# sonniki/image-captioning-with-external-knowledge

Hardware: AMD Instinct MI355X
Metric: decode_steps_per_sec (higher is better)
Workload: dtype f32 (3xbf16 split products, fp32 accumulate); 1 GPU; cfg2: geo variant, per-GPU batch 64 x 20 decode positions, 14x14x2048 features, K=20 knowledge rows, vocab 10000; global_batch=64, graph=True, collective_backend=none, split_allreduce=False, parallelism=dp1 (one flat-bucket all-reduce per step)

## Files before the change

### image-captioning-with-external-knowledge_amd/csrc/attention_mfma.hip

```cpp
#include <algorithm>

#include "attention_mfma.h"

#ifdef ICK_ATTN_STAMPS
__device__ unsigned long long ick_attn_stamps[4][16];
#define ICK_ASTAMP(kern, i)                                                                   \
    do {                                                                                      \
        if (threadIdx.x == 0 && blockIdx.x == 0 && blockIdx.y == 0) ick_attn_stamps[kern][i] = __builtin_readcyclecounter(); \
    } while (0)
extern "C" int ick_debug_read_attn_stamps(unsigned long long* out) {
    return (int)hipMemcpyFromSymbol(out, HIP_SYMBOL(ick_attn_stamps), sizeof(ick_attn_stamps));
}
#else
#define ICK_ASTAMP(kern, i)
#endif

namespace ick {
namespace {

constexpr int DHP = 32;
constexpr int QLD = DHP + 4;

__device__ __forceinline__ float4 mask_cols(float4 x, int c0, int dh) {
    x.x = c0 + 0 < dh ? x.x : 0.f; x.y = c0 + 1 < dh ? x.y : 0.f;
    x.z = c0 + 2 < dh ? x.z : 0.f; x.w = c0 + 3 < dh ? x.w : 0.f;
    return x;
}

__device__ __forceinline__ int wave_id_of(unsigned tid) { return __builtin_amdgcn_readfirstlane((int)(tid >> 6)); }

__device__ __forceinline__ f32x4 mfma4(const float4& a, const float4& b, f32x4 c) {
    c = __builtin_amdgcn_mfma_f32_16x16x4f32(a.x, b.x, c, 0, 0, 0);
    c = __builtin_amdgcn_mfma_f32_16x16x4f32(a.y, b.y, c, 0, 0, 0);
// ... 161 lines not shown
        }
        if (lq == 0) rsum[wave * NQ + 16 * qt + li] = sum[qt];
    }
    ICK_ASTAMP(SK, 6);
    __syncthreads();
    ICK_ASTAMP(SK, 7);
#pragma unroll
    for (int qt = 0; qt < NQT; ++qt)
#pragma unroll
        for (int jt = 0; jt < 2; ++jt)
            *reinterpret_cast<f32x4*>(Ored + ((wave * NQT + qt) * 2 + jt) * 256 + lane * 4) = oacc[qt][jt];
    if (tid < NQ) {
        const float s = (rsum[tid] + rsum[NQ + tid]) + (rsum[2 * NQ + tid] + rsum[3 * NQ + tid]);
        stat[NQ + tid] = s > 0.f ? 1.f / s : 0.f;
        if (p.lse && tid < T) p.lse[((int64_t)b * p.H + h) * T + tid] = stat[tid] + __logf(s);
    }
    __syncthreads();
    for (int tt = wave; tt < NQT * 2; tt += 4) {
        const int qt = tt >> 1, jt = tt & 1;
        f32x4 o = {0.f, 0.f, 0.f, 0.f};
#pragma unroll
        for (int w = 0; w < 4; ++w) o += *reinterpret_cast<const f32x4*>(Ored + ((w * NQT + qt) * 2 + jt) * 256 + lane * 4);
        const int query = 16 * qt + li;
        if (query < T) {
            const float inv = stat[NQ + query];
            float* orow = p.O + (int64_t)b * p.o_bs + (int64_t)query * p.o_ts + h * dh;
            const int j0 = 16 * jt + 4 * lq;
#pragma unroll
            for (int r = 0; r < 4; ++r)
                if (j0 + r < dh) orow[j0 + r] = o[r] * inv;
        }
    }
    ICK_ASTAMP(SK, 8);
}

template <int NQT, int MAXT>
__global__ __launch_bounds__(256) void attn_bwd_mfma_kernel(ick_attn_bwd_args p, int SP, bool st2) {
    chain_priority_bwd();
    [[maybe_unused]] constexpr int SK = MAXT > 1 ? 3 : 2;
    ICK_ASTAMP(SK, 0);
    constexpr int NQ = NQT * 16;
    constexpr int TLD = NQ + 4;
    extern __shared__ __attribute__((aligned(16))) float smem[];
    const int TR = (p.T + 3) & ~3;
    float* dSs = smem;
    float* Qs = dSs + TR * SP;
    float* Gs = Qs + NQ * QLD;
    float* Qt = Gs + NQ * QLD;
    float* Gt = Qt + DHP * TLD;
    float* Ls = Gt + DHP * TLD;
    float* Dl = Ls + NQ;
    float* Kw = Dl + NQ + (wave_id_of(threadIdx.x)) * (16 * QLD);
    float* dQp = Qs;

    const int b = blockIdx.x, h = blockIdx.y;
    const int tid = threadIdx.x, lane = tid & 63, wave = tid >> 6;
    const int li = lane & 15, lq = lane >> 4;
    const int T = p.T, S = p.S, dh = p.dh;
    const int nkt = (S + 15) >> 4;
    const Dropout drop = make_dropout(p.drop_p, epoch_seed(p.drop_seed, p.drop_epoch), p.drop_site);
    const float* qb = p.Q + (int64_t)b * p.q_bs + (int64_t)h * p.q_hs;
    const float* kb = p.K + (int64_t)b * p.k_bs + (int64_t)h * p.k_hs;
    const float* vb = p.V + (int64_t)b * p.v_bs + (int64_t)h * p.v_hs;
    const float* ob = p.O + (int64_t)b * p.o_bs + h * dh;
    const float* gb = p.dO + (int64_t)b * p.o_bs + h * dh;

    constexpr int QIT = (NQ * 8 + 255) / 256;
    float4 qx[QIT];
#pragma unroll
    for (int it = 0; it < QIT; ++it) {
        const int f = tid + 256 * it;
        const int t = f >> 3, c = f & 7;
        qx[it] = *reinterpret_cast<const float4*>(qb + (int64_t)(t < T ? t : 0) * DHP + 4 * c);
    }
    const float lse_v = p.lse[((int64_t)b * p.H + h) * T + (tid < T ? tid : 0)];
    float gv[NQT * 2], ov[NQT * 2];
#pragma unroll
    for (int it = 0; it < NQT * 2; ++it) {
        const int f = tid + 256 * it;
        const int t = f >> 5, j = f & 31;
        const bool ok = t < T && j < dh;
        const int64_t at = ok ? (int64_t)t * p.o_ts + j : 0;
        gv[it] = gb[at];
        ov[it] = ob[at];
    }
    float4 kf[MAXT][2], vf[MAXT][2];
#pragma unroll
    for (int i = 0; i < MAXT; ++i) {
        const int key = 16 * (wave + 4 * i) + li;
        const int64_t ro = (int64_t)(key < S ? key : 0) * DHP + 4 * lq;
#pragma unroll
        for (int t = 0; t < 2; ++t) {
            kf[i][t] = *reinterpret_cast<const float4*>(kb + ro + 16 * t);
            vf[i][t] = *reinterpret_cast<const float4*>(vb + ro + 16 * t);
        }
    }
    ICK_ASTAMP(SK, 1);
#pragma unroll
    for (int it = 0; it < QIT; ++it) {
        const int f = tid + 256 * it;
        const int t = f >> 3, c = f & 7;
        if (f < NQ * 8) {
            const float4 x = mask_cols(qx[it], 4 * c, t < T ? dh : 0);
            *reinterpret_cast<float4*>(Qs + t * QLD + 4 * c) = x;
            Qt[(4 * c + 0) * TLD + t] = x.x; Qt[(4 * c + 1) * TLD + t] = x.y;
            Qt[(4 * c + 2) * TLD + t] = x.z; Qt[(4 * c + 3) * TLD + t] = x.w;
        }
    }
#pragma unroll
    for (int it = 0; it < NQT * 2; ++it) {
        const int f = tid + 256 * it;
        const int t = f >> 5, j = f & 31;
        const bool ok = t < T && j < dh;
        const float g = ok ? gv[it] : 0.f, o = ok ? ov[it] : 0.f;
        Gs[t * QLD + j] = g;
        Gt[j * TLD + t] = g;
        float d = g * o;
        d += __shfl_xor(d, 1, 64); d += __shfl_xor(d, 2, 64); d += __shfl_xor(d, 4, 64);
        d += __shfl_xor(d, 8, 64); d += __shfl_xor(d, 16, 64);
        if (j == 0) Dl[t] = d;
    }
    if (tid < NQ) Ls[tid] = tid < T ? lse_v : 0.f;
    ICK_ASTAMP(SK, 2);
    __syncthreads();
    ICK_ASTAMP(SK, 3);

    f32x4 dq[NQT][2];
#pragma unroll
    for (int qt = 0; qt < NQT; ++qt)
#pragma unroll
        for (int jt = 0; jt < 2; ++jt) dq[qt][jt] = f32x4{0.f, 0.f, 0.f, 0.f};
#pragma unroll
    for (int i = 0; i < MAXT; ++i) {
        const int kt = wave + 4 * i;
        if (kt >= nkt) continue;
        const int key = 16 * kt + li;
        const bool kok = key < S;
#pragma unroll
        for (int t = 0; t < 2; ++t) {
            kf[i][t] = mask_cols(kf[i][t], 16 * t + 4 * lq, kok ? dh : 0);
            vf[i][t] = mask_cols(vf[i][t], 16 * t + 4 * lq, kok ? dh : 0);
        }
#pragma unroll
        for (int t = 0; t < 2; ++t) *reinterpret_cast<float4*>(Kw + li * QLD + 16 * t + 4 * lq) = kf[i][t];
        f32x4 dvt[2] = {{0.f, 0.f, 0.f, 0.f}, {0.f, 0.f, 0.f, 0.f}};
        f32x4 dkt[2] = {{0.f, 0.f, 0.f, 0.f}, {0.f, 0.f, 0.f, 0.f}};
#pragma unroll
        for (int qt = 0; qt < NQT; ++qt) {
            f32x4 s = {0.f, 0.f, 0.f, 0.f}, dp = {0.f, 0.f, 0.f, 0.f};
#pragma unroll
            for (int t = 0; t < 2; ++t) {
                const float4 qa = *reinterpret_cast<const float4*>(Qs + (16 * qt + li) * QLD + 16 * t + 4 * lq);
                const float4 ga = *reinterpret_cast<const float4*>(Gs + (16 * qt + li) * QLD + 16 * t + 4 * lq);
                s = mfma4(qa, kf[i][t], s);
                dp = mfma4(ga, vf[i][t], dp);
            }
            const float4 l4 = *reinterpret_cast<const float4*>(Ls + 16 * qt + 4 * lq);
            const float4 d4 = *reinterpret_cast<const float4*>(Dl + 16 * qt + 4 * lq);
            const float lr[4] = {l4.x, l4.y, l4.z, l4.w}, dr[4] = {d4.x, d4.y, d4.z, d4.w};
            float pd[4], ds[4];
#pragma unroll
            for (int r = 0; r < 4; ++r) {
                const int query = 16 * qt + 4 * lq + r;
                float pr = __expf(s[r] * p.scale - lr[r]);
                if (!kok || query >= T || (p.causal && key > p.q_pos0 + query)) pr = 0.f;
                float mk = 1.f;
                if (drop.on()) mk = drop.mask((uint32_t)((b * p.H + h) * T + query) * (uint32_t)S + (uint32_t)key);
                ds[r] = pr * (dp[r] * mk - dr[r]) * p.scale;
                pd[r] = pr * mk;
                if (query < T) dSs[query * SP + key] = ds[r];
            }
            const float4 pf = make_float4(pd[0], pd[1], pd[2], pd[3]);
            const float4 df = make_float4(ds[0], ds[1], ds[2], ds[3]);
#pragma unroll
            for (int jt = 0; jt < 2; ++jt) {
                const float4 gt = *reinterpret_cast<const float4*>(Gt + (16 * jt + li) * TLD + 16 * qt + 4 * lq);
                const float4 qt4 = *reinterpret_cast<const float4*>(Qt + (16 * jt + li) * TLD + 16 * qt + 4 * lq);
                dvt[jt] = mfma4(gt, pf, dvt[jt]);
                dkt[jt] = mfma4(qt4, df, dkt[jt]);
            }
        }
        __builtin_amdgcn_fence(__ATOMIC_RELEASE, "wavefront");
        __builtin_amdgcn_wave_barrier();
        {
            float4 kq[2];
#pragma unroll
            for (int jt = 0; jt < 2; ++jt) {
                const float* kc = Kw + (4 * lq) * QLD + 16 * jt + li;
                kq[jt] = make_float4(kc[0], kc[QLD], kc[2 * QLD], kc[3 * QLD]);
            }
#pragma unroll
            for (int qt = 0; qt < NQT; ++qt) {
                const float4 da = *reinterpret_cast<const float4*>(dSs + (16 * qt + li) * SP + 16 * kt + 4 * lq);
#pragma unroll
                for (int jt = 0; jt < 2; ++jt) dq[qt][jt] = mfma4(da, kq[jt], dq[qt][jt]);
            }
        }
        __builtin_amdgcn_wave_barrier();
        if (kok) {
            float* dvr = p.dV + (int64_t)b * p.dv_bs + (int64_t)key * p.dv_ss + h * dh;
            float* dkr = p.dK + (int64_t)b * p.dk_bs + (int64_t)key * p.dk_ss + h * dh;
#pragma unroll
            for (int jt = 0; jt < 2; ++jt) {
                const int j0 = 16 * jt + 4 * lq;
                if (st2) {
                    if (j0 + 1 < dh) {
                        *reinterpret_cast<float2*>(dvr + j0) = make_float2(dvt[jt][0], dvt[jt][1]);
                        *reinterpret_cast<float2*>(dkr + j0) = make_float2(dkt[jt][0], dkt[jt][1]);
                    }
                    if (j0 + 3 < dh) {
                        *reinterpret_cast<float2*>(dvr + j0 + 2) = make_float2(dvt[jt][2], dvt[jt][3]);
                        *reinterpret_cast<float2*>(dkr + j0 + 2) = make_float2(dkt[jt][2], dkt[jt][3]);
                    }
                } else {
#pragma unroll
                    for (int r = 0; r < 4; ++r)
                        if (j0 + r < dh) { dvr[j0 + r] = dvt[jt][r]; dkr[j0 + r] = dkt[jt][r]; }
                }
            }
        }
    }
    ICK_ASTAMP(SK, 4);
    __syncthreads();
    ICK_ASTAMP(SK, 5);
#pragma unroll
    for (int qt = 0; qt < NQT; ++qt)
#pragma unroll
        for (int jt = 0; jt < 2; ++jt)
            *reinterpret_cast<f32x4*>(dQp + ((wave * NQT + qt) * 2 + jt) * 256 + lane * 4) = dq[qt][jt];
    __syncthreads();
    for (int tt = wave; tt < NQT * 2; tt += 4) {
        const int qt = tt >> 1, jt = tt & 1;
        const int j = 16 * jt + li;
        f32x4 acc = {0.f, 0.f, 0.f, 0.f};
#pragma unroll
        for (int w = 0; w < 4; ++w) acc += *reinterpret_cast<const f32x4*>(dQp + ((w * NQT + qt) * 2 + jt) * 256 + lane * 4);
        if (j < dh) {
#pragma unroll
            for (int r = 0; r < 4; ++r) {
                const int query = 16 * qt + 4 * lq + r;
                if (query < T) p.dQ[(int64_t)b * p.dq_bs + (int64_t)query * p.dq_ts + h * dh + j] = acc[r];
            }
        }
    }
    ICK_ASTAMP(SK, 6);
}

template <int NQT, int MAXT>
int launch_fwd(const ick_attn_args& a, int SP, hipStream_t s) {
    const size_t fl = std::max<size_t>((size_t)DHP * SP, 4 * NQT * 2 * 256) + (size_t)NQT * 16 * QLD + 10 * NQT * 16;
    if (fl * sizeof(float) > 150 * 1024) return kAttnMfmaUnsupported;
    auto kern = attn_fwd_mfma_kernel<NQT, MAXT>;
    static LdsAttrOnce attr;
    if (int e = attr.ensure((const void*)kern, 160 * 1024)) return e;
    hipLaunchKernelGGL(kern, dim3(a.H, a.B), dim3(256), fl * sizeof(float), s, a, SP);
    ICK_LAUNCH_RET();
}

template <int NQT, int MAXT>
int launch_bwd(const ick_attn_bwd_args& a, int SP, hipStream_t s) {
    constexpr int NQ = NQT * 16;
    const size_t tr = (size_t)((a.T + 3) & ~3);
    const size_t fl = std::max(tr * SP + 2 * (size_t)NQ * QLD + 2 * (size_t)DHP * (NQ + 4) + 2 * NQ + 4 * 16 * QLD,
                               (size_t)NQ * SP + 64);
    if (fl * sizeof(float) > 150 * 1024) return kAttnMfmaUnsupported;
    auto kern = attn_bwd_mfma_kernel<NQT, MAXT>;
    static LdsAttrOnce attr;
    if (int e = attr.ensure((const void*)kern, 160 * 1024)) return e;
    const bool st2 = a.dh % 2 == 0 && a.dk_bs % 2 == 0 && a.dk_ss % 2 == 0 && a.dv_bs % 2 == 0 && a.dv_ss % 2 == 0 &&
// ... 49 lines not shown
```

### image-captioning-with-external-knowledge_amd/csrc/common.h

```cpp
#pragma once
#include <hip/hip_runtime.h>
#include <stdint.h>
#include <stdlib.h>

#include "ick_amd.h"

namespace ick {

using f32x4 = __attribute__((ext_vector_type(4))) float;

constexpr int kWave = 64;

inline int ceil_div(int64_t a, int64_t b) { return (int)((a + b - 1) / b); }

extern int g_deterministic;
inline bool deterministic() {
    if (g_deterministic < 0) {
        const char* e = getenv("ICK_DETERMINISTIC");
        g_deterministic = (e && e[0] && e[0] != '0') ? 1 : 0;
    }
    return g_deterministic == 1;
}

#define ICK_CHECK_ARG(cond)          \
// ... 94 lines not shown
    uint32_t thr, seed, site;
    float scale;
    __device__ __forceinline__ bool on() const { return thr != 0u; }
    __device__ __forceinline__ float mask(uint32_t idx) const { return drop_hash(seed, site, idx) >= thr ? scale : 0.f; }
};
__host__ __device__ __forceinline__ Dropout make_dropout(float p, uint32_t seed, uint32_t site) {
    Dropout d{0u, seed, site, 1.f};
    if (p > 0.f) {
        d.thr = (uint32_t)fminf(p * 4294967296.f, 4294967040.f);
        d.scale = 1.f / (1.f - p);
    }
    return d;
}
__device__ __forceinline__ uint32_t epoch_seed(uint32_t seed, const uint32_t* epoch) {
    if (epoch == nullptr) return seed;
#if defined(__HIP_DEVICE_COMPILE__)
    uint32_t v;
    asm volatile("s_load_dword %0, %1, 0x0\n\ts_waitcnt lgkmcnt(0)" : "=s"(v) : "s"(epoch) : "memory");
    return seed + v;
#else
    return seed + *epoch;
#endif
}
__device__ __forceinline__ int device_bound(int host, const int32_t* dev) {
    if (dev == nullptr) return host;
#if defined(__HIP_DEVICE_COMPILE__)
    int v;
    asm volatile("s_load_dword %0, %1, 0x0\n\ts_waitcnt lgkmcnt(0)" : "=s"(v) : "s"(dev) : "memory");
    return min(host, max(v, 0));
#else
    return host;
#endif
}
__device__ __forceinline__ int clamp_row(int64_t v, int n) {
    return (int)(v < 0 ? 0 : (v >= (int64_t)n ? (int64_t)n - 1 : v));
}
constexpr int kRuleHistMax = 128;
__device__ __forceinline__ uint4 rule_words(const int32_t* words) {
    if (words == nullptr) return make_uint4(0u, 0u, 0u, 0u);
#if defined(__HIP_DEVICE_COMPILE__)
    uint64_t w01;
    uint32_t w2;
    asm volatile("s_load_dwordx2 %0, %2, 0x0\n\ts_load_dword %1, %2, 0x8\n\ts_waitcnt lgkmcnt(0)"
                 : "=&s"(w01), "=&s"(w2) : "s"(words) : "memory");
    return make_uint4((uint32_t)w01, (uint32_t)(w01 >> 32), w2, 0u);
#else
    return make_uint4((uint32_t)words[0], (uint32_t)words[1], (uint32_t)words[2], (uint32_t)words[3]);
#endif
}

template <typename Tok>
__device__ __forceinline__ void mark_bans(const Tok* hist, int t, int n, int m, int end_token, uint32_t* bits, int c0,
                                          int nwords, int* hs) {
    const int tid = threadIdx.x, nt = blockDim.x;
    for (int w = tid; w < nwords; w += nt) bits[w] = 0u;
    if (n > 0)
        for (int p = tid; p < t; p += nt) hs[p] = (int)hist[p];
    __syncthreads();
    if (n > 0) {
        for (int p = n - 1 + tid; p < t; p += nt) {
            bool match = true;
            for (int j = 1; j < n; ++j) match = match && hs[p - j] == hs[t - j];
            const int c = hs[p] - c0;
            if (match && c >= 0 && c < 32 * nwords) atomicOr(&bits[c >> 5], 1u << (c & 31));
        }
    }
// ... 41 lines not shown
```

### image-captioning-with-external-knowledge_amd/lib.py

```python
import ctypes as C
import os

_PKG = os.path.dirname(os.path.abspath(__file__))
LIB_PATH = os.path.join(_PKG, "libick_amd.so")
if os.environ.get("ICK_LIB_PATH"):
    LIB_PATH = os.environ["ICK_LIB_PATH"]

ICK_GEO, ICK_KNOWLEDGE, ICK_NEWS = 0, 1, 2
VARIANT_ID = {"geo": ICK_GEO, "knowledge": ICK_KNOWLEDGE, "news": ICK_NEWS}
GEMM_RELU, GEMM_ACCUM, GEMM_ATOMIC, GEMM_COLSUM_ONLY = 1, 2, 4, 16

vp = C.c_void_p
i32 = C.c_int32
i64 = C.c_int64
f32 = C.c_float
u32 = C.c_uint32


class GemmArgs(C.Structure):
    _fields_ = [
        ("A", vp), ("B", vp), ("C", vp), ("bias", vp),
        ("M", i32), ("N", i32), ("K", i32),
        ("a_rs", i64), ("a_ks", i64), ("a_grp", i32), ("a_gs", i64), ("a_gmap", vp),
        ("b_rs", i64), ("b_ks", i64),
# ... 64 lines not shown

class AdamBlock(C.Structure):
    _fields_ = [("item", i32), ("tn", i32), ("tk", i32), ("cnt4", i32), ("off4", i64), ("copy", vp)]


class LrSchedule(C.Structure):
    _fields_ = [("kind", i32), ("warmup", i32), ("total", i32), ("min_ratio", f32)]


OPT_WORDS = 8
LR_KINDS = {"constant": 0, "inverse_sqrt": 1, "cosine": 2, "linear": 3}


class AttnArgs(C.Structure):
    _fields_ = [
        ("Q", vp), ("K", vp), ("V", vp), ("O", vp), ("lse", vp),
        ("B", i32), ("H", i32), ("T", i32), ("S", i32), ("dh", i32),
        ("q_bs", i64), ("q_hs", i64), ("q_ts", i64), ("k_bs", i64), ("k_hs", i64), ("k_ss", i64),
        ("v_bs", i64), ("v_hs", i64), ("v_ss", i64), ("o_bs", i64), ("o_ts", i64),
        ("scale", f32), ("causal", i32), ("q_pos0", i32), ("kv_len", vp),
        ("drop_p", f32), ("drop_seed", u32), ("drop_site", u32), ("drop_epoch", vp),
    ]


class AttnBwdArgs(C.Structure):
    _fields_ = [
        ("Q", vp), ("K", vp), ("V", vp), ("O", vp), ("dO", vp), ("lse", vp), ("dQ", vp), ("dK", vp), ("dV", vp),
        ("B", i32), ("H", i32), ("T", i32), ("S", i32), ("dh", i32),
        ("q_bs", i64), ("q_hs", i64), ("q_ts", i64), ("k_bs", i64), ("k_hs", i64), ("k_ss", i64),
        ("v_bs", i64), ("v_hs", i64), ("v_ss", i64), ("o_bs", i64), ("o_ts", i64),
        ("dq_bs", i64), ("dq_ts", i64), ("dk_bs", i64), ("dk_ss", i64), ("dv_bs", i64), ("dv_ss", i64),
        ("scale", f32), ("causal", i32), ("q_pos0", i32),
        ("drop_p", f32), ("drop_seed", u32), ("drop_site", u32), ("drop_epoch", vp),
    ]


class DecodeLayer(C.Structure):
    _fields_ = [(n, vp) for n in ("sa_in_w", "sa_in_b", "sa_out_wt", "sa_out_b", "n1_g", "n1_b",
                                  "ca_in_w", "ca_in_b", "ca_out_wt", "ca_out_b", "n2_g", "n2_b",
                                  "w1", "b1", "w2t", "b2", "n3_g", "n3_b", "self_k", "self_v", "cross_k", "cross_v")]


MAX_LAYERS = 8


class DecodeCtx(C.Structure):
    _fields_ = ([(n, i32) for n in ("R", "rows_per_sample", "d", "H", "FF", "layers", "S", "max_len", "V", "K", "F",
                                    "end_token", "pad_token")] +
                [("ln_eps", f32), ("emb_scale", f32), ("kv_bs", i64), ("scores_ld", i64),
                 ("layer", DecodeLayer * MAX_LAYERS)] +
                [(n, vp) for n in ("anc", "wv", "bv", "we", "be", "wf", "bf", "ee", "fe", "gate", "eib", "word_emb", "pe",
                                   "x0", "xa", "xb", "xc", "p1", "p2", "p3", "hfin", "hv", "ptr", "cand", "scores",
                                   "output", "hist", "finished", "n_done", "next_token", "next_mask", "cap_buf", "sel_state")])


class BeamState(C.Structure):
    _fields_ = [(n, vp) for n in ("cum", "fin", "seq_in", "seq_out", "anc_in", "anc_out", "cap_in", "cap_out", "rec")] + \
               [("start_token", i32)]


class SampleState(C.Structure):
    _fields_ = [(n, vp) for n in ("seed", "temp_top_p", "top_k", "log_prob")]


class DecodeRules(C.Structure):
    _fields_ = [(n, vp) for n in ("words", "lp", "len")]
# ... 136 lines not shown
```

### image-captioning-with-external-knowledge_amd/ops.py

```python
import contextlib
import ctypes as C
import gc
import math
import os

import torch

from . import lib as L


def _p(t):
    return None if t is None else t.data_ptr()


def _stream():
    return torch.cuda.current_stream().cuda_stream


def _f32c(t, name):
    if t.dtype != torch.float32 or not t.is_cuda:
        raise L.IckError("%s must be a float32 device tensor (got %s on %s)" % (name, t.dtype, t.device))
    return t


# ... 841 lines not shown
    N = rouge_l.shape[0] if rouge_l.dim() == 1 else -1
    if N < 1 or tuple(counts.shape) != (N, 10) or tuple(pointers.shape) != (N, 3):
        raise L.IckError("caption_metric_sums needs counts (N, 10), rouge_l (N,) and pointers (N, 3), N >= 1")
    dev = counts.device
    if out is None:
        out = (torch.empty(14, device=dev, dtype=torch.int64), torch.empty(1, device=dev, dtype=torch.float64))
    sums, rouge_sum = out
    assert sums.shape == (14,) and sums.dtype == torch.int64 and sums.is_contiguous()
    assert rouge_sum.shape == (1,) and rouge_sum.dtype == torch.float64
    L.check(L.load().ick_caption_metric_sums(_p(counts), _p(rouge_l), _p(pointers), N, _p(sums), _p(rouge_sum),
                                             _p(sums[13:14]), _stream()), "ick_caption_metric_sums")
    return sums, rouge_sum


def attention_bwd_buffer(shape, T, S, dh, device):
    if L.load().ick_attention_bwd_overwrites(T, S, dh):
        return torch.empty(shape, device=device, dtype=torch.float32)
    return torch.zeros(shape, device=device, dtype=torch.float32)


ATTN_PLAN_KEYS = ("mfma", "nqt", "maxt", "dhp", "tq", "chunks", "overwrites")


def attention_plan(direction, T, S, dh, head_major=True):
    out = (C.c_int32 * len(ATTN_PLAN_KEYS))()
    rc = L.load_raw().ick_attention_plan({"fwd": 0, "bwd": 1}[direction], T, S, dh, int(head_major), out)
    if rc == -1:
        return None
    L.check(rc, "ick_attention_plan")
    return dict(zip(ATTN_PLAN_KEYS, (int(v) for v in out)))


def attention_heads_bwd(q, kv, O, dO, lse, dQ, dK, dV, H, dh, T, S, q_seg=0, k_seg=0, v_seg=1, causal=False,
                        drop=None, q_pos0=0):
    B = q.shape[0]
    Tq, Sa = q.shape[3], kv.shape[3]
    hp = q.shape[4]
    assert kv.shape[4] == hp
    a = L.AttnBwdArgs()
    a.Q = q.data_ptr() + 4 * (q_seg * H * Tq * hp)
    a.K = kv.data_ptr() + 4 * (k_seg * H * Sa * hp)
    a.V = kv.data_ptr() + 4 * (v_seg * H * Sa * hp)
    a.O, a.dO, a.lse = _p(O), _p(dO), _p(lse)
    a.dQ, a.dK, a.dV = _p(dQ), _p(dK), _p(dV)
    a.B, a.H, a.T, a.S, a.dh = B, H, T, S, dh
    a.q_bs, a.q_hs, a.q_ts = q.stride(0), Tq * hp, hp
    a.k_bs, a.k_hs, a.k_ss = kv.stride(0), Sa * hp, hp
    a.v_bs, a.v_hs, a.v_ss = kv.stride(0), Sa * hp, hp
    a.o_bs, a.o_ts = O.stride(0), O.stride(1)
    a.dq_bs, a.dq_ts = dQ.stride(0), dQ.stride(1)
    a.dk_bs, a.dk_ss = dK.stride(0), dK.stride(1)
    a.dv_bs, a.dv_ss = dV.stride(0), dV.stride(1)
    a.scale = 1.0 / math.sqrt(dh)
    a.causal, a.q_pos0 = int(causal), q_pos0
    _drop(a, drop)
    L.check(L.load().ick_attention_bwd(C.byref(a), _stream()), "ick_attention_bwd")


def layernorm_bwd(dy, x, res, gamma, mean, rstd, dgamma, dbeta, drop=None):
    d = x.shape[-1]
    rows = x.numel() // d
    dz = torch.empty_like(x)
    dxd = torch.empty_like(x)
    rpb = L.load().ick_layernorm_bwd_rows_per_block()
    part = torch.empty((rows + rpb - 1) // rpb, 2 * d, device=x.device, dtype=torch.float32)
    L.check(L.load().ick_layernorm_bwd(_p(dy), _p(x), _p(res), _p(gamma), _p(mean), _p(rstd), _p(dz), None, None,
                                       rows, d, _p(dxd), *_dargs(drop), _p(part), _stream()), "ick_layernorm_bwd")

    if SIDE is not None:
        SIDE.flush()
    ln_partials_reduce(part, dgamma, dbeta)
    return dz, dxd


def ln_partials_reduce(part, dgamma, dbeta):
    d = part.shape[1] // 2
    adjacent = dbeta.data_ptr() == dgamma.data_ptr() + 4 * d
    if SIDE is not None:
        if adjacent:
            SIDE.add_problem(colsum_problem(part, dgamma), part)
        else:
            SIDE.add_problem(colsum_problem(part[:, :d], dgamma), part)
            SIDE.add_problem(colsum_problem(part[:, d:], dbeta), part)
    elif adjacent:
        colsum(part, dgamma, n_out=2 * d)
    else:
        colsum(part[:, :d], dgamma)
        colsum(part[:, d:], dbeta)
# ... 350 lines not shown
```

### image-captioning-with-external-knowledge_amd/training.py

```python
import functools
import math
import os
import weakref

import torch

from . import dp, ops
from .decoder import DropSites
from .lib import IckError
from .weights import DerivedWeights, first_stage, vocab_planes_wanted


class Tape:

    def __init__(self):
        self.enc_layers = {}
        self.dec_layers = []
        self.misc = {}


def _p(x):
    return x.detach()


# ... 219 lines not shown
                _lin_bwd(grads, dqkv.view(M, 3 * d), t["x"].view(M, d), layer.self_attn.in_proj_weight,
                         layer.self_attn.in_proj_bias, need_dx=False)
                dz, g0, w0p = dz_out, dqkv.view(M, 3 * d), pkb[(tag, li, "siT")]
            else:
                dx = _lin_bwd(grads, dqkv.view(M, 3 * d), t["x"].view(M, d), layer.self_attn.in_proj_weight,
                              layer.self_attn.in_proj_bias, dx=dz_out, acc=True).view(B, T, d)
                if ops.SIDE is not None:
                    ops.SIDE.flush_group_here()
        return dx
    for layer, t in zip(reversed(layers), reversed(tapes)):
        B, T, _ = t["x"].shape
        M = B * T
        dz, do2 = ops.layernorm_bwd(dx, t["o2"], t["x1"], _p(layer.norm2.weight), t["m2"], t["r2"],
                                    _g(grads, layer.norm2.weight), _g(grads, layer.norm2.bias), drop=t["d2"])
        dpre = _lin_bwd(grads, do2.view(M, d), t["f"].view(M, -1), layer.linear2.weight, layer.linear2.bias,
                        gate=t["f"].view(M, -1), gate_scale=_keep_scale(t["d_ff"]))
        dx1 = _lin_bwd(grads, dpre, t["x1"].view(M, d), layer.linear1.weight, layer.linear1.bias, dx=dz.view(M, d),
                       acc=True)
        dz, do1 = ops.layernorm_bwd(dx1.view(B, T, d), t["o1"], t["x"], _p(layer.norm1.weight), t["m1"], t["r1"],
                                    _g(grads, layer.norm1.weight), _g(grads, layer.norm1.bias), drop=t["d1"])
        dsa = _lin_bwd(grads, do1.view(M, d), t["sa"].view(M, d), layer.self_attn.out_proj.weight,
                       layer.self_attn.out_proj.bias)
        dqkv = ops.attention_bwd_buffer((B, T, 3 * d), T, T, d // H, dx.device)
        ops.attention_heads_bwd(t["qkv"], t["qkv"], t["sa"], dsa.view(B, T, d), t["lse"], dqkv[:, :, :d],
                                dqkv[:, :, d:2 * d], dqkv[:, :, 2 * d:], H, d // H, T, T, 0, 1, 2, drop=t["d_att"])
        dx = _lin_bwd(grads, dqkv.view(M, 3 * d), t["x"].view(M, d), layer.self_attn.in_proj_weight,
                      layer.self_attn.in_proj_bias, dx=dz.view(M, d), acc=True).view(B, T, d)
        if ops.SIDE is not None:
            ops.SIDE.flush_group()
    return dx


def _decoder_layer_bwd_chain(dec, li, layer, t, state, dkv_rows, kv, S, grads, pkb, mem2=None, mem_t_ps=None,
                             valid=None):
    H, d = dec.num_heads, dec.emb_dim
    dh = d // H
    B, T, _ = t["x"].shape
    M = B * T
    dev = t["x"].device
    dz, g0, w0p = state
    n3 = _norm_args(t, 3, t["x2"], layer.norm3, grads, M, d, dev)
    n2 = _norm_args(t, 2, t["x1"], layer.norm2, grads, M, d, dev)
    dpre = torch.empty(M, layer.linear1.out_features, device=dev, dtype=torch.float32)
    dca = torch.empty(M, d, device=dev, dtype=torch.float32)
    dz_a = torch.empty(M, d, device=dev, dtype=torch.float32)
    ops.rowchain_bwd(M, d, n3, pkb[("d", li, "coT")], dca, dz_a, g0=g0, w0p=w0p, dzin=dz,
                     ffn=dict(w1p=pkb[("d", li, "l2T")], w2p=pkb[("d", li, "l1T")], act=t["f"],
                              gate_scale=_keep_scale(t["d_ff"]), t_out=dpre), norm2=n2)
    if ops.SIDE is not None:
        ops.SIDE.flush()
    ops.ln_partials_reduce(n3["part"], _g(grads, layer.norm3.weight), _g(grads, layer.norm3.bias))
    ops.ln_partials_reduce(n2["part"], _g(grads, layer.norm2.weight), _g(grads, layer.norm2.bias))
    _lin_bwd(grads, n3["do"], t["f"].view(M, -1), layer.linear2.weight, layer.linear2.bias, need_dx=False,
             valid=valid)
    _lin_bwd(grads, dpre, t["x2"].view(M, d), layer.linear1.weight, layer.linear1.bias, need_dx=False, valid=valid)
    _lin_bwd(grads, n2["do"], t["ca"].view(M, d), layer.multihead_attn.out_proj.weight,
             layer.multihead_attn.out_proj.bias, need_dx=False, valid=valid)
    if ops.SIDE is not None:
        ops.SIDE.flush_group()
    dq = torch.empty(B, T, d, device=dev, dtype=torch.float32)
    c0 = 2 * li * d
    ops.attention_heads_bwd(t["qc"], kv, t["ca"], dca.view(B, T, d), t["lse_c"], dq, dkv_rows[:, :, c0:c0 + d],
                            dkv_rows[:, :, c0 + d:c0 + 2 * d], H, dh, T, S, 0, 2 * li, 2 * li + 1, drop=t["d_ca"])
    if ops.SIDE is not None:
        ops.SIDE.flush()
    if mem2 is not None:
        _kv_proj_param_grads(layer, li, dkv_rows, mem2, grads, d, mem_t_ps)
    n1 = _norm_args(t, 1, t["x"], layer.norm1, grads, M, d, dev)
    dsa = torch.empty(M, d, device=dev, dtype=torch.float32)
    dz_b = torch.empty(M, d, device=dev, dtype=torch.float32)
    ops.rowchain_bwd(M, d, n1, pkb[("d", li, "soT")], dsa, dz_b, g0=dq.view(M, d), w0p=pkb[("d", li, "cqT")], dzin=dz_a)
    if ops.SIDE is not None:
        ops.SIDE.flush()
    ops.ln_partials_reduce(n1["part"], _g(grads, layer.norm1.weight), _g(grads, layer.norm1.bias))
    _lin_bwd(grads, dq.view(M, d), t["x1"].view(M, d), layer.multihead_attn.in_proj_weight,
             layer.multihead_attn.in_proj_bias, w_rows=slice(0, d), need_dx=False, valid=valid)
    _lin_bwd(grads, n1["do"], t["sa"].view(M, d), layer.self_attn.out_proj.weight, layer.self_attn.out_proj.bias,
             need_dx=False, valid=valid)
    dqkv = ops.attention_bwd_buffer((B, T, 3 * d), T, T, dh, dev)
    ops.attention_heads_bwd(t["qkv"], t["qkv"], t["sa"], dsa.view(B, T, d), t["lse_s"], dqkv[:, :, :d],
                            dqkv[:, :, d:2 * d], dqkv[:, :, 2 * d:], H, dh, T, T, 0, 1, 2, causal=True,
                            drop=t["d_sa"])
    if li > 0:
        _lin_bwd(grads, dqkv.view(M, 3 * d), t["x"].view(M, d), layer.self_attn.in_proj_weight,
                 layer.self_attn.in_proj_bias, need_dx=False, valid=valid)
        out = (dz_b, dqkv.view(M, 3 * d), pkb[("d", li, "siT")])
    else:
        dx0 = _lin_bwd(grads, dqkv.view(M, 3 * d), t["x"].view(M, d), layer.self_attn.in_proj_weight,
                       layer.self_attn.in_proj_bias, dx=dz_b, acc=True, valid=valid).view(B, T, d)
        out = (dx0, None, None)
    if ops.SIDE is not None:
        ops.SIDE.flush_group()
    return out


def _decoder_layer_bwd(dec, li, layer, t, dx, dkv_rows, kv, S, grads, mem2=None, mem_t_ps=None, valid=None):
    H, d = dec.num_heads, dec.emb_dim
    dh = d // H
    B, T, _ = t["x"].shape
    M = B * T
    dz, do3 = ops.layernorm_bwd(dx, t["o3"], t["x2"], _p(layer.norm3.weight), t["m3"], t["r3"],
                                _g(grads, layer.norm3.weight), _g(grads, layer.norm3.bias), drop=t["d3"])
    dpre = _lin_bwd(grads, do3.view(M, d), t["f"].view(M, -1), layer.linear2.weight, layer.linear2.bias,
                    gate=t["f"].view(M, -1), gate_scale=_keep_scale(t["d_ff"]),
                    valid=valid)
    dx2 = _lin_bwd(grads, dpre, t["x2"].view(M, d), layer.linear1.weight, layer.linear1.bias, dx=dz.view(M, d),
                   acc=True, valid=valid)
    dz, do2 = ops.layernorm_bwd(dx2.view(B, T, d), t["o2"], t["x1"], _p(layer.norm2.weight), t["m2"], t["r2"],
                                _g(grads, layer.norm2.weight), _g(grads, layer.norm2.bias), drop=t["d2"])
    dca = _lin_bwd(grads, do2.view(M, d), t["ca"].view(M, d), layer.multihead_attn.out_proj.weight,
                   layer.multihead_attn.out_proj.bias, valid=valid)
    dq = torch.empty(B, T, d, device=dx.device, dtype=torch.float32)
    c0 = 2 * li * d
    ops.attention_heads_bwd(t["qc"], kv, t["ca"], dca.view(B, T, d), t["lse_c"], dq, dkv_rows[:, :, c0:c0 + d],
                            dkv_rows[:, :, c0 + d:c0 + 2 * d], H, dh, T, S, 0, 2 * li, 2 * li + 1, drop=t["d_ca"])
    if mem2 is not None:
        _kv_proj_param_grads(layer, li, dkv_rows, mem2, grads, d, mem_t_ps)
    dx1 = _lin_bwd(grads, dq.view(M, d), t["x1"].view(M, d), layer.multihead_attn.in_proj_weight,
                   layer.multihead_attn.in_proj_bias, w_rows=slice(0, d), dx=dz.view(M, d), acc=True, valid=valid)
    dz, do1 = ops.layernorm_bwd(dx1.view(B, T, d), t["o1"], t["x"], _p(layer.norm1.weight), t["m1"], t["r1"],
                                _g(grads, layer.norm1.weight), _g(grads, layer.norm1.bias), drop=t["d1"])
    dsa = _lin_bwd(grads, do1.view(M, d), t["sa"].view(M, d), layer.self_attn.out_proj.weight,
                   layer.self_attn.out_proj.bias, valid=valid)
    dqkv = ops.attention_bwd_buffer((B, T, 3 * d), T, T, dh, dx.device)
    ops.attention_heads_bwd(t["qkv"], t["qkv"], t["sa"], dsa.view(B, T, d), t["lse_s"], dqkv[:, :, :d],
                            dqkv[:, :, d:2 * d], dqkv[:, :, 2 * d:], H, dh, T, T, 0, 1, 2, causal=True,
                            drop=t["d_sa"])
    dx0 = _lin_bwd(grads, dqkv.view(M, 3 * d), t["x"].view(M, d), layer.self_attn.in_proj_weight,
                   layer.self_attn.in_proj_bias, dx=dz.view(M, d), acc=True, valid=valid).view(B, T, d)
    if ops.SIDE is not None:
        ops.SIDE.flush_group()
    return dx0


def _kv_proj_param_grads(layer, li, dkv_rows, mem2, grads, d, mem_t_ps=None):
    gw, gb = _g(grads, layer.multihead_attn.in_proj_weight), _g(grads, layer.multihead_attn.in_proj_bias)
    rows = mem2.shape[0]
    sl = dkv_rows.view(rows, -1)[:, 2 * li * d:(2 * li + 2) * d]
    if gw is not None:
        if mem_t_ps is not None:
            split = max(1, min(32, 160 // (((2 * d + 127) // 128) * ((d + 79) // 80)), rows // 256))
            wg = ops.gemm_args(sl, mem2, gw[d:], 2 * d, d, rows, 1, sl.stride(0), 1, d, d, atomic=True, split_k=split,
                               b_ps=mem_t_ps)
            extra = [] if gb is None else [ops.colsum_problem(sl, gb[d:], split_k=max(1, min(16, rows // 512)))]
        else:
            wg = ops.gemm_args(sl, mem2, gw[d:], 2 * d, d, rows, 1, sl.stride(0), 1, d, d, atomic=True,
                               split_k=1 if ops.is_deterministic() else 16,
                               colsum_a=None if gb is None else gb[d:])
            extra = []
        if ops.SIDE is not None:
            ops.SIDE.add_problem(wg, dkv_rows, mem2, mem_t_ps)
            for e in extra:
                ops.SIDE.add_problem(e, dkv_rows)
        else:
            ops.gemm_grouped([wg] + extra)
    elif gb is not None:
        ops.colsum(sl, gb[d:])


def _memory_t_presplit(m, B, S, d):
# ... 74 lines not shown
    def late(self):
        if self.side is not None and getattr(self, "joined", False):
            self.retired = self.side
            self.side = ops.SideStream()
        self._run(True)


def _backward_phases(dec, tape, dscores, grads, want_image_grad=False):
    m = tape.misc
    d, V, H = dec.emb_dim, dec.vocab_size, dec.num_heads
    h, ee, fe = m["h"], m["ee"], m["fe"]
    grads = dict(grads)
    for prm in unique_parameters(dec):
        if id(prm) not in grads and prm is not dec.word_embedding.weight:
            grads[id(prm)] = torch.zeros_like(prm)
    B, L, _ = h.shape
    P, K, Fn, S = m["P"], m["K"], m["Fn"], m["S"]
    M = B * L
    Vx = dscores.shape[2]
    dsc2 = dscores.view(M, Vx)
    dev = h.device
    pre = m.get("prezero") or {}

    def zeroed(name, like):
        t = pre.get(name)
        return t if t is not None and t.shape == like.shape else torch.zeros_like(like)

    dee = zeroed("dee", ee)
    dfe = zeroed("dfe", fe) if fe is not None else None
    hv = m["hv"] if dec.has_facts else h
    dhv0 = pre.get("dhv")
    pack = m.get("pack")
    valid = pack if os.environ.get("ICK_NO_VALID_ROW_WGRAD", "0") in ("", "0") and not ops.is_deterministic() else None
    hv_t_ps = _rows_t_presplit(hv.view(M, d), pack) if _g(grads, dec.fc_vocab.weight) is not None else None
    if pack is not None:
        if dhv0 is None or dhv0.shape != (M, d):
            dhv0 = torch.zeros(M, d, device=dev, dtype=torch.float32)
        dhv = _lin_bwd(grads, dsc2[:, :V], hv.view(M, d), dec.fc_vocab.weight, dec.fc_vocab.bias, dx=dhv0, acc=True,
                       group_now=True, wt_ps=m.get("vocab_t_ps"), xt_ps=hv_t_ps, pack=pack).view(B, L, d)
    elif dhv0 is not None and dhv0.shape == (M, d) and not ops.is_deterministic():
        dhv = _lin_bwd(grads, dsc2[:, :V], hv.view(M, d), dec.fc_vocab.weight, dec.fc_vocab.bias, dx=dhv0, acc=True,
                       group_now=True, wt_ps=m.get("vocab_t_ps"), xt_ps=hv_t_ps).view(B, L, d)
    else:
        dhv = _lin_bwd(grads, dsc2[:, :V], hv.view(M, d), dec.fc_vocab.weight, dec.fc_vocab.bias,
                       group_now=True, wt_ps=m.get("vocab_t_ps"), xt_ps=hv_t_ps).view(B, L, d)
    if dec.has_facts:
        dh = ops.mul(dhv, m["gate"])
        dgate = ops.mul(dhv, h)
        gw, gb = _g(grads, dec.fc_predicate.weight), _g(grads, dec.fc_predicate.bias)
        if gw is not None:
            ops.context_gate_bwd(m["captions"], m["facts"], dgate, gw, gb, K, V, mode=0)
    else:
        dh = dhv

    def gbuf(param):
        return _g(grads, param)

    ops.pointer_scores_bwd(dscores, V, h, ee, _p(dec.fc_entity.weight), None, dh, dee, gbuf(dec.fc_entity.weight),
                           gbuf(dec.fc_entity.bias), pack=pack)
    if dec.has_facts:
        ops.pointer_scores_bwd(dscores, V + K, h, fe, _p(dec.fc_fact.weight), m["eib"], dh, dfe,
                               gbuf(dec.fc_fact.weight), gbuf(dec.fc_fact.bias), pack=pack)
    layers = list(dec.transformer_decoder.layers)
    nseg = 2 * len(layers)
    dkv_rows = ops.attention_bwd_buffer((B, S, nseg * d), L, S, d // H, dev)
    dx = dh
    ops.stamp("bwd: head done")
    pkb = m.get("pkb")
    mem_t_ps = _memory_t_presplit(m, B, S, d)
    if pkb is not None:
        state = (dh.view(M, d), None, None)
        for li in reversed(range(len(layers))):
            state = _decoder_layer_bwd_chain(dec, li, layers[li], tape.dec_layers[li], state, dkv_rows, m["kv"], S,
                                             grads, pkb, mem2=m["mem"].view(B * S, d), mem_t_ps=mem_t_ps,
                                             valid=valid)
            ops.stamp("bwd: decoder layer %d done" % li)
        dx = state[0]
    else:
        for li in reversed(range(len(layers))):
            dx = _decoder_layer_bwd(dec, li, layers[li], tape.dec_layers[li], dx, dkv_rows, m["kv"], S, grads,
                                    mem2=m["mem"].view(B * S, d), mem_t_ps=mem_t_ps, valid=valid)
            ops.stamp("bwd: decoder layer %d done" % li)
    yield
    nctx = K + Fn
    dkv_ctx = dkv_rows[:, P:]
    fuse_ctx = pkb is not None and ops.rowchain_bwd_supported(nseg * d, d, 0)
    dctx = None
    if not fuse_ctx:
        ksplit = max(1, min(8, (nseg * d) // 450)) if B * nctx * d <= 1280 * 512 else 1
        if ops.is_deterministic():
            ksplit = 1
        dctx = (torch.zeros if ksplit > 1 else torch.empty)(B, nctx, d, device=dev, dtype=torch.float32)
        ops.gemm_raw(dkv_ctx, m["wkv"], dctx, B * nctx, d, nseg * d, nseg * d, 1, 1, d, d, a_grp=nctx,
                     a_gs=S * nseg * d, atomic=ksplit > 1, split_k=ksplit)
    if want_image_grad:
        d_img = torch.empty(B, P, d, device=dev, dtype=torch.float32)
        ops.gemm_raw(dkv_rows, m["wkv"], d_img, B * P, d, nseg * d, nseg * d, 1, 1, d, d, a_grp=P, a_gs=S * nseg * d)
        m["d_img"] = d_img
    ops.stamp("bwd: context gradient ready")
    dee_enc = _context_encoder_bwd(dec, dec.transformer_encoder_entities, tape.enc_layers["entities"],
                                   None if fuse_ctx else dctx[:, :K].contiguous(), grads, pkb=pkb, tag="e",
                                   g_first=(dkv_ctx[:, :K], pkb[("kv", "T")]) if fuse_ctx else None)
    ops.stamp("bwd: entity context encoder done")
    dee += dee_enc
    if dec.has_facts:
        dfe_enc = _context_encoder_bwd(dec, dec.transformer_encoder_facts, tape.enc_layers["facts"],
                                       None if fuse_ctx else dctx[:, K:].contiguous(), grads, pkb=pkb, tag="f",
                                       g_first=(dkv_ctx[:, K:], pkb[("kv", "T")]) if fuse_ctx else None)
        dfe += dfe_enc
    gword = _g(grads, dec.word_embedding.weight)
    ops.caption_embed_bwd(dx, m["captions"], m["masks"], gword, dee, dfe, V, dec.word_map["<pad>"], math.sqrt(d),
                          drop=m["d_pos"])
    if dec.has_facts:
        ops.fact_encode_bwd(dfe, m["facts"], dee, gbuf(dec.predicate_embedding.weight))
# ... 578 lines not shown
```

### include/ick_amd.h

```cpp
#ifndef ICK_AMD_H
#define ICK_AMD_H

#include <stdint.h>

#ifdef __cplusplus
extern "C" {
#endif

#define ICK_OK 0
#define ICK_EINVAL (-1)
#define ICK_EALIGN (-2)
#define ICK_EWORKSPACE (-3)

#define ICK_MAX_LAYERS 8

int ick_version(void);
int ick_set_deterministic(int on);
int ick_get_deterministic(void);
int ick_device_info(int* num_cu, int* wave_size, char* arch_name, int arch_name_len);

typedef struct {
    const float* A; const float* B; float* C; const float* bias;
    int32_t M, N, K;
    int64_t a_rs, a_ks; int32_t a_grp; int64_t a_gs; const int32_t* a_gmap;
// ... 241 lines not shown
int ick_packed_ce_weighted(const float* scores, int64_t ld, const int64_t* captions_sorted, const int32_t* decode_len,
                           const float* weights, int32_t B, int32_t L, int32_t Vx, int32_t pad_token,
                           float* row_loss , float* loss_sum, float* count, float* dscores,
                           void* stream);
int ick_samples_to_captions(const int64_t* tokens, int32_t R, int32_t T, int32_t V, int32_t K, int32_t has_facts,
                            int32_t start_token, int32_t end_token, int32_t pad_token, int64_t* captions, int64_t* masks,
                            int64_t* lengths, void* stream);

int ick_cider_d(const int64_t* cand, int32_t N, int32_t T, const int64_t* refs, int32_t B, int32_t M, int32_t Lr,
                const uint32_t* df_keys, const int32_t* df_count, int32_t U, float log_ref_len, float sigma,
                int32_t start_token, int32_t end_token, int32_t pad_token, const int32_t* ignore, int32_t n_ignore,
                int32_t mode, const int32_t* image_index, int32_t num_samples, float* rewards, float* advantages,
                void* stream);

int ick_caption_metrics(const int64_t* cand, int32_t N, int32_t T, const int64_t* refs, int32_t B, int32_t M, int32_t Lr,
                        int32_t start_token, int32_t end_token, int32_t pad_token, const int32_t* ignore,
                        int32_t n_ignore, int32_t pointer_base, double beta, int32_t mode, const int32_t* image_index,
                        int32_t num_samples, const float* base_rewards, const float* weights, int32_t* counts,
                        float* bleu, float* rouge_l, int32_t* pointers, float* rewards, float* advantages, void* stream);

int ick_caption_metric_sums(const int32_t* counts, const float* rouge_l, const int32_t* pointers, int32_t N,
                            int64_t* sums, double* rouge_sum, int64_t* captions, void* stream);


typedef struct {
    const float* Q; const float* K; const float* V; const float* O; const float* dO; const float* lse;
    float* dQ; float* dK; float* dV;
    int32_t B, H, T, S, dh;
    int64_t q_bs, q_hs, q_ts, k_bs, k_hs, k_ss, v_bs, v_hs, v_ss, o_bs, o_ts;
    int64_t dq_bs, dq_ts, dk_bs, dk_ss, dv_bs, dv_ss;
    float scale; int32_t causal; int32_t q_pos0;
    float drop_p; uint32_t drop_seed, drop_site;
    const uint32_t* drop_epoch;
} ick_attn_bwd_args;
int ick_attention_bwd(const ick_attn_bwd_args* args, void* stream);
int ick_attention_bwd_overwrites(int32_t T, int32_t S, int32_t dh);
int ick_attention_plan(int32_t dir, int32_t T, int32_t S, int32_t dh, int32_t head_major, int32_t* out);

int ick_layernorm_bwd_rows_per_block(void);
int ick_layernorm_bwd(const float* dy, const float* x, const float* res, const float* gamma, const float* mean,
                      const float* rstd, float* dz, float* dgamma, float* dbeta, int64_t rows, int32_t d,
                      float* dx_drop ,
                      float drop_p, uint32_t drop_seed, uint32_t drop_site, const uint32_t* drop_epoch, float* partials,
                      void* stream);
int ick_relu_bwd(const float* dy, const float* act, float* dx, int64_t n, float scale ,
                 void* stream);
int ick_colsum(const float* a, int64_t M, int32_t N, int64_t ld, float* out, void* stream);
int ick_caption_embed_bwd(const float* dx, const int64_t* captions, const int64_t* masks, float* dword,
                          float* dee, float* dfe, int32_t B, int32_t L, int32_t K, int32_t F, int32_t V,
                          int32_t d, int32_t pad_token, float scale, float drop_p, uint32_t drop_seed,
                          uint32_t drop_site, const uint32_t* drop_epoch, void* stream);
int ick_pointer_scores_bwd(const float* ds, int64_t ds_ld, int32_t col0, const float* h, const float* ctx,
                           const float* w, const float* ind, float* dh, float* dctx, float* dw, float* dbias,
                           int32_t B, int32_t T, int32_t Kc, int32_t d, void* stream);
int ick_entity_encode_bwd(int32_t variant, const float* dee, const float* entities, int32_t ent_cols,
                          const float* ee, const float* word_emb, int32_t vocab, float* dtype_emb,
                          int32_t ntypes, float* dword, int32_t B, int32_t K, int32_t d, void* stream);
int ick_fact_encode_bwd(const float* dfe, const int64_t* facts, float* dee, float* dpred, int32_t num_pred,
                        int32_t B, int32_t K, int32_t F, int32_t d, void* stream);
int ick_context_gate_bwd(const int64_t* captions, const int64_t* facts, const float* dgate, float* dw,
                         float* dbias, int32_t B, int32_t L, int32_t T, int32_t K, int32_t F, int32_t V,
                         int32_t num_pred, int32_t d, int32_t mode, void* stream);
int ick_adam_clamp(float* p, float* g, float* m, float* v, int64_t n, float gscale, float clip, float lr,
                   float beta1, float beta2, float eps, int32_t step, const uint32_t* step_ptr,
                   const float* gscale_den, void* stream);
typedef struct ick_adam_item {
// ... 73 lines not shown
```

Before: 805,600 decode-steps/s.

## Skip padded query tiles in attention backward using per-sample decode lengths

Passes a per-batch valid query length into the MFMA attention backward kernel. The kernel reads it with the epoch seed and dispatches a compile-time count of live query tiles, so the staging, S/dP MFMAs, dQ accumulation and reduction skip tiles that hold only padded positions. The aim is to cut wasted work on short captions in the decoder's self- and cross-attention backward. It adds more template instantiations, which grows code size, plus an extra scalar load per block.

Result: no change. 805,700 decode-steps/s (median of 2 runs) (+0.0%).

```diff
diff --git a/image-captioning-with-external-knowledge_amd/csrc/attention_mfma.hip b/image-captioning-with-external-knowledge_amd/csrc/attention_mfma.hip
--- a/image-captioning-with-external-knowledge_amd/csrc/attention_mfma.hip
+++ b/image-captioning-with-external-knowledge_amd/csrc/attention_mfma.hip
@@ -1,4 +1,5 @@
 #include <algorithm>
+#include <type_traits>
 
 #include "attention_mfma.h"
 
@@ -226,6 +227,12 @@
         }
     }
     ICK_ASTAMP(SK, 8);
+}
+
+template <int N, class F>
+__device__ __forceinline__ void live_tiles(int n, F& f) {
+    if (n >= N) f(std::integral_constant<int, N>{});
+    else if constexpr (N > 0) live_tiles<N - 1>(n, f);
 }
 
 template <int NQT, int MAXT>
@@ -252,7 +259,11 @@
     const int li = lane & 15, lq = lane >> 4;
     const int T = p.T, S = p.S, dh = p.dh;
     const int nkt = (S + 15) >> 4;
-    const Dropout drop = make_dropout(p.drop_p, epoch_seed(p.drop_seed, p.drop_epoch), p.drop_site);
+    uint32_t seed = p.drop_seed;
+    int q_rows = T;
+    epoch_seed_and_bound(seed, p.drop_epoch, q_rows, p.q_len ? p.q_len + b : nullptr);
+    const int n_live = (q_rows + 15) >> 4;
+    const Dropout drop = make_dropout(p.drop_p, seed, p.drop_site);
     const float* qb = p.Q + (int64_t)b * p.q_bs + (int64_t)h * p.q_hs;
     const float* kb = p.K + (int64_t)b * p.k_bs + (int64_t)h * p.k_hs;
     const float* vb = p.V + (int64_t)b * p.v_bs + (int64_t)h * p.v_hs;
@@ -294,7 +305,7 @@
     for (int it = 0; it < QIT; ++it) {
         const int f = tid + 256 * it;
         const int t = f >> 3, c = f & 7;
-        if (f < NQ * 8) {
+        if (f < NQ * 8 && t < 16 * n_live) {
             const float4 x = mask_cols(qx[it], 4 * c, t < T ? dh : 0);
             *reinterpret_cast<float4*>(Qs + t * QLD + 4 * c) = x;
             Qt[(4 * c + 0) * TLD + t] = x.x; Qt[(4 * c + 1) * TLD + t] = x.y;
@@ -303,6 +314,7 @@
     }
 #pragma unroll
     for (int it = 0; it < NQT * 2; ++it) {
+        if (it >= 2 * n_live) continue;
         const int f = tid + 256 * it;
         const int t = f >> 5, j = f & 31;
         const bool ok = t < T && j < dh;
@@ -314,7 +326,7 @@
         d += __shfl_xor(d, 8, 64); d += __shfl_xor(d, 16, 64);
         if (j == 0) Dl[t] = d;
     }
-    if (tid < NQ) Ls[tid] = tid < T ? lse_v : 0.f;
+    if (tid < 16 * n_live) Ls[tid] = tid < T ? lse_v : 0.f;
     ICK_ASTAMP(SK, 2);
     __syncthreads();
     ICK_ASTAMP(SK, 3);
@@ -324,6 +336,8 @@
     for (int qt = 0; qt < NQT; ++qt)
 #pragma unroll
         for (int jt = 0; jt < 2; ++jt) dq[qt][jt] = f32x4{0.f, 0.f, 0.f, 0.f};
+    auto key_tiles = [&](auto nl) {
+    constexpr int NL = decltype(nl)::value;
 #pragma unroll
     for (int i = 0; i < MAXT; ++i) {
         const int kt = wave + 4 * i;
@@ -340,7 +354,7 @@
         f32x4 dvt[2] = {{0.f, 0.f, 0.f, 0.f}, {0.f, 0.f, 0.f, 0.f}};
         f32x4 dkt[2] = {{0.f, 0.f, 0.f, 0.f}, {0.f, 0.f, 0.f, 0.f}};
 #pragma unroll
-        for (int qt = 0; qt < NQT; ++qt) {
+        for (int qt = 0; qt < NL; ++qt) {
             f32x4 s = {0.f, 0.f, 0.f, 0.f}, dp = {0.f, 0.f, 0.f, 0.f};
 #pragma unroll
             for (int t = 0; t < 2; ++t) {
@@ -384,7 +398,7 @@
                 kq[jt] = make_float4(kc[0], kc[QLD], kc[2 * QLD], kc[3 * QLD]);
             }
 #pragma unroll
-            for (int qt = 0; qt < NQT; ++qt) {
+            for (int qt = 0; qt < NL; ++qt) {
                 const float4 da = *reinterpret_cast<const float4*>(dSs + (16 * qt + li) * SP + 16 * kt + 4 * lq);
 #pragma unroll
                 for (int jt = 0; jt < 2; ++jt) dq[qt][jt] = mfma4(da, kq[jt], dq[qt][jt]);
@@ -414,21 +428,27 @@
             }
         }
     }
+    };
+    live_tiles<NQT>(n_live, key_tiles);
     ICK_ASTAMP(SK, 4);
     __syncthreads();
     ICK_ASTAMP(SK, 5);
 #pragma unroll
-    for (int qt = 0; qt < NQT; ++qt)
+    for (int qt = 0; qt < NQT; ++qt) {
+        if (qt >= n_live) continue;
 #pragma unroll
         for (int jt = 0; jt < 2; ++jt)
             *reinterpret_cast<f32x4*>(dQp + ((wave * NQT + qt) * 2 + jt) * 256 + lane * 4) = dq[qt][jt];
+    }
     __syncthreads();
     for (int tt = wave; tt < NQT * 2; tt += 4) {
         const int qt = tt >> 1, jt = tt & 1;
         const int j = 16 * jt + li;
         f32x4 acc = {0.f, 0.f, 0.f, 0.f};
-#pragma unroll
-        for (int w = 0; w < 4; ++w) acc += *reinterpret_cast<const f32x4*>(dQp + ((w * NQT + qt) * 2 + jt) * 256 + lane * 4);
+        if (qt < n_live) {
+#pragma unroll
+            for (int w = 0; w < 4; ++w) acc += *reinterpret_cast<const f32x4*>(dQp + ((w * NQT + qt) * 2 + jt) * 256 + lane * 4);
+        }
         if (j < dh) {
 #pragma unroll
             for (int r = 0; r < 4; ++r) {
diff --git a/image-captioning-with-external-knowledge_amd/csrc/common.h b/image-captioning-with-external-knowledge_amd/csrc/common.h
--- a/image-captioning-with-external-knowledge_amd/csrc/common.h
+++ b/image-captioning-with-external-knowledge_amd/csrc/common.h
@@ -150,6 +150,21 @@
     return host;
 #endif
 }
+__device__ __forceinline__ void epoch_seed_and_bound(uint32_t& seed, const uint32_t* epoch, int& bound, const int32_t* dev) {
+#if defined(__HIP_DEVICE_COMPILE__)
+    if (epoch != nullptr && dev != nullptr) {
+        uint32_t e;
+        int v;
+        asm volatile("s_load_dword %0, %2, 0x0\n\ts_load_dword %1, %3, 0x0\n\ts_waitcnt lgkmcnt(0)"
+                     : "=&s"(e), "=&s"(v) : "s"(epoch), "s"(dev) : "memory");
+        seed += e;
+        bound = min(bound, max(v, 0));
+        return;
+    }
+#endif
+    seed = epoch_seed(seed, epoch);
+    bound = device_bound(bound, dev);
+}
 __device__ __forceinline__ int clamp_row(int64_t v, int n) {
     return (int)(v < 0 ? 0 : (v >= (int64_t)n ? (int64_t)n - 1 : v));
 }
diff --git a/image-captioning-with-external-knowledge_amd/lib.py b/image-captioning-with-external-knowledge_amd/lib.py
--- a/image-captioning-with-external-knowledge_amd/lib.py
+++ b/image-captioning-with-external-knowledge_amd/lib.py
@@ -120,6 +120,7 @@
         ("dq_bs", i64), ("dq_ts", i64), ("dk_bs", i64), ("dk_ss", i64), ("dv_bs", i64), ("dv_ss", i64),
         ("scale", f32), ("causal", i32), ("q_pos0", i32),
         ("drop_p", f32), ("drop_seed", u32), ("drop_site", u32), ("drop_epoch", vp),
+        ("q_len", vp),
     ]
 
 
diff --git a/image-captioning-with-external-knowledge_amd/ops.py b/image-captioning-with-external-knowledge_amd/ops.py
--- a/image-captioning-with-external-knowledge_amd/ops.py
+++ b/image-captioning-with-external-knowledge_amd/ops.py
@@ -897,7 +897,7 @@
 
 
 def attention_heads_bwd(q, kv, O, dO, lse, dQ, dK, dV, H, dh, T, S, q_seg=0, k_seg=0, v_seg=1, causal=False,
-                        drop=None, q_pos0=0):
+                        drop=None, q_pos0=0, q_len=None):
     B = q.shape[0]
     Tq, Sa = q.shape[3], kv.shape[3]
     hp = q.shape[4]
@@ -919,6 +919,10 @@
     a.scale = 1.0 / math.sqrt(dh)
     a.causal, a.q_pos0 = int(causal), q_pos0
     _drop(a, drop)
+    if q_len is not None:
+        if q_len.dtype != torch.int32 or not q_len.is_cuda or not q_len.is_contiguous() or q_len.numel() != B:
+            raise L.IckError("attention_heads_bwd: q_len must be a contiguous (B,) int32 device tensor")
+        a.q_len = _p(q_len)
     L.check(L.load().ick_attention_bwd(C.byref(a), _stream()), "ick_attention_bwd")
 
 
diff --git a/image-captioning-with-external-knowledge_amd/training.py b/image-captioning-with-external-knowledge_amd/training.py
--- a/image-captioning-with-external-knowledge_amd/training.py
+++ b/image-captioning-with-external-knowledge_amd/training.py
@@ -275,7 +275,7 @@
 
 
 def _decoder_layer_bwd_chain(dec, li, layer, t, state, dkv_rows, kv, S, grads, pkb, mem2=None, mem_t_ps=None,
-                             valid=None):
+                             valid=None, q_len=None):
     H, d = dec.num_heads, dec.emb_dim
     dh = d // H
     B, T, _ = t["x"].shape
@@ -304,7 +304,8 @@
     dq = torch.empty(B, T, d, device=dev, dtype=torch.float32)
     c0 = 2 * li * d
     ops.attention_heads_bwd(t["qc"], kv, t["ca"], dca.view(B, T, d), t["lse_c"], dq, dkv_rows[:, :, c0:c0 + d],
-                            dkv_rows[:, :, c0 + d:c0 + 2 * d], H, dh, T, S, 0, 2 * li, 2 * li + 1, drop=t["d_ca"])
+                            dkv_rows[:, :, c0 + d:c0 + 2 * d], H, dh, T, S, 0, 2 * li, 2 * li + 1, drop=t["d_ca"],
+                            q_len=q_len)
     if ops.SIDE is not None:
         ops.SIDE.flush()
     if mem2 is not None:
@@ -323,7 +324,7 @@
     dqkv = ops.attention_bwd_buffer((B, T, 3 * d), T, T, dh, dev)
     ops.attention_heads_bwd(t["qkv"], t["qkv"], t["sa"], dsa.view(B, T, d), t["lse_s"], dqkv[:, :, :d],
                             dqkv[:, :, d:2 * d], dqkv[:, :, 2 * d:], H, dh, T, T, 0, 1, 2, causal=True,
-                            drop=t["d_sa"])
+                            drop=t["d_sa"], q_len=q_len)
     if li > 0:
         _lin_bwd(grads, dqkv.view(M, 3 * d), t["x"].view(M, d), layer.self_attn.in_proj_weight,
                  layer.self_attn.in_proj_bias, need_dx=False, valid=valid)
@@ -337,7 +338,8 @@
     return out
 
 
-def _decoder_layer_bwd(dec, li, layer, t, dx, dkv_rows, kv, S, grads, mem2=None, mem_t_ps=None, valid=None):
+def _decoder_layer_bwd(dec, li, layer, t, dx, dkv_rows, kv, S, grads, mem2=None, mem_t_ps=None, valid=None,
+                       q_len=None):
     H, d = dec.num_heads, dec.emb_dim
     dh = d // H
     B, T, _ = t["x"].shape
@@ -356,7 +358,8 @@
     dq = torch.empty(B, T, d, device=dx.device, dtype=torch.float32)
     c0 = 2 * li * d
     ops.attention_heads_bwd(t["qc"], kv, t["ca"], dca.view(B, T, d), t["lse_c"], dq, dkv_rows[:, :, c0:c0 + d],
-                            dkv_rows[:, :, c0 + d:c0 + 2 * d], H, dh, T, S, 0, 2 * li, 2 * li + 1, drop=t["d_ca"])
+                            dkv_rows[:, :, c0 + d:c0 + 2 * d], H, dh, T, S, 0, 2 * li, 2 * li + 1, drop=t["d_ca"],
+                            q_len=q_len)
     if mem2 is not None:
         _kv_proj_param_grads(layer, li, dkv_rows, mem2, grads, d, mem_t_ps)
     dx1 = _lin_bwd(grads, dq.view(M, d), t["x1"].view(M, d), layer.multihead_attn.in_proj_weight,
@@ -368,7 +371,7 @@
     dqkv = ops.attention_bwd_buffer((B, T, 3 * d), T, T, dh, dx.device)
     ops.attention_heads_bwd(t["qkv"], t["qkv"], t["sa"], dsa.view(B, T, d), t["lse_s"], dqkv[:, :, :d],
                             dqkv[:, :, d:2 * d], dqkv[:, :, 2 * d:], H, dh, T, T, 0, 1, 2, causal=True,
-                            drop=t["d_sa"])
+                            drop=t["d_sa"], q_len=q_len)
     dx0 = _lin_bwd(grads, dqkv.view(M, 3 * d), t["x"].view(M, d), layer.self_attn.in_proj_weight,
                    layer.self_attn.in_proj_bias, dx=dz.view(M, d), acc=True, valid=valid).view(B, T, d)
     if ops.SIDE is not None:
@@ -509,6 +512,7 @@
     dhv0 = pre.get("dhv")
     pack = m.get("pack")
     valid = pack if os.environ.get("ICK_NO_VALID_ROW_WGRAD", "0") in ("", "0") and not ops.is_deterministic() else None
+    q_len = pack.decode_len if pack is not None and os.environ.get("ICK_NO_VALID_ROW_ATTN", "0") in ("", "0") else None
     hv_t_ps = _rows_t_presplit(hv.view(M, d), pack) if _g(grads, dec.fc_vocab.weight) is not None else None
     if pack is not None:
         if dhv0 is None or dhv0.shape != (M, d):
@@ -550,13 +554,13 @@
         for li in reversed(range(len(layers))):
             state = _decoder_layer_bwd_chain(dec, li, layers[li], tape.dec_layers[li], state, dkv_rows, m["kv"], S,
                                              grads, pkb, mem2=m["mem"].view(B * S, d), mem_t_ps=mem_t_ps,
-                                             valid=valid)
+                                             valid=valid, q_len=q_len)
             ops.stamp("bwd: decoder layer %d done" % li)
         dx = state[0]
     else:
         for li in reversed(range(len(layers))):
             dx = _decoder_layer_bwd(dec, li, layers[li], tape.dec_layers[li], dx, dkv_rows, m["kv"], S, grads,
-                                    mem2=m["mem"].view(B * S, d), mem_t_ps=mem_t_ps, valid=valid)
+                                    mem2=m["mem"].view(B * S, d), mem_t_ps=mem_t_ps, valid=valid, q_len=q_len)
             ops.stamp("bwd: decoder layer %d done" % li)
     yield
     nctx = K + Fn
diff --git a/include/ick_amd.h b/include/ick_amd.h
--- a/include/ick_amd.h
+++ b/include/ick_amd.h
@@ -297,6 +297,7 @@
     float scale; int32_t causal; int32_t q_pos0;
     float drop_p; uint32_t drop_seed, drop_site;
     const uint32_t* drop_epoch;
+    const int32_t* q_len;
 } ick_attn_bwd_args;
 int ick_attention_bwd(const ick_attn_bwd_args* args, void* stream);
 int ick_attention_bwd_overwrites(int32_t T, int32_t S, int32_t dh);
```
